# liznerski/eoe

Hardware: AMD Instinct MI355X
Metric: train images/sec, CLIP ViT-B/32 + HSC, 224x224 (higher is better)
Workload: dtype fp16; 1 GPU; CLIP ViT-B/32 (12 layers) + Linear(512,256) + HSC, full fine-tune, Adam lr 1e-4 wd 1e-3, 224x224, 128 normal + 128 OE images per GPU per step; global_batch=256, parallelism=dp1, launch=eager, weight-gradient launches on a side stream under the dgrad chain, arithmetic=16-bit MFMA operands, fp32 accumulate

## Files before the change

### eoe_amd/csrc/gemm.hip

```cpp
#include "gemm_common.h"
#include <stdlib.h>
#include <map>
#include <mutex>
#include <type_traits>

unsigned long long* g_stamp_buf = nullptr;
extern int g_tn_flags;
extern int g_vit_side_stream;
extern int g_attn_flags;
extern int g_tn256_launches;
extern int g_parity_flags;
int eoe_launch_nt256(const void* gemm_p, int dtype, int epi, int mi, hipStream_t s);
bool eoe_w8_applies(const void* gemm_p, int epi);
int eoe_launch_w8(const void* gemm_p, int dtype, int epi, hipStream_t s);
bool eoe_w8_streamk(const void* gemm_p);

namespace {
extern int g_nt_flags;


template <typename T, int EPI, int NI, int FLAGS, int GATHER = 0>
__global__ __launch_bounds__(512, 2) void gemm_nt_kernel(GemmP p) {
    extern __shared__ __attribute__((aligned(16))) char smem[];
    const int tid = threadIdx.x, lane = tid & 63, wave = tid >> 6;
// ... 660 lines not shown
        EOE_NT128_CASE(EOE_EPI_GELU_BWD)
        default: return eoe_set_error(EOE_ERR_ARG, "gemm_nt: unknown epilogue %d", epi);
    }
#undef EOE_NT128_CASE
    EOE_CHECK_LAUNCH("gemm_nt128");
    return finish_colsum(p, epi, MI, s);
}

template <typename T>
int launch_nt128w(const GemmP& p, int epi, hipStream_t s) {
    const int tiles = cdiv(p.M, 160) * cdiv(p.N, 256);
#define EOE_NT128W_CASE(E)                                                                  \
    case E:                                                                                 \
        { static bool once = (hipFuncSetAttribute((const void*)gemm_nt128w_kernel<T, E>, hipFuncAttributeMaxDynamicSharedMemorySize, SMEMW_BYTES), true); (void)once; } \
        hipLaunchKernelGGL((gemm_nt128w_kernel<T, E>), dim3(tiles), dim3(256), SMEMW_BYTES, s, p); \
        break;
    switch (epi) {
        EOE_NT128W_CASE(EOE_EPI_NONE)
        EOE_NT128W_CASE(EOE_EPI_GELU)
        EOE_NT128W_CASE(EOE_EPI_RESIDUAL)
        EOE_NT128W_CASE(EOE_EPI_GELU_BWD)
        default: return eoe_set_error(EOE_ERR_ARG, "gemm_nt: unknown epilogue %d", epi);
    }
#undef EOE_NT128W_CASE
    EOE_CHECK_LAUNCH("gemm_nt128w");
    return finish_colsum(p, epi, 5, s);
}

template <typename T>
int launch_nt128_auto(const GemmP& p, int epi, hipStream_t s) {
    const int slots = 2 * num_cus();
    const long t4 = (long)cdiv(p.M, 128) * cdiv(p.N, 128), t5 = (long)cdiv(p.M, 160) * cdiv(p.N, 128);
    const long c4 = (t4 + slots - 1) / slots * 128, c5 = (t5 + slots - 1) / slots * 160;
    const bool five = (g_nt_flags & 32) || (!(g_nt_flags & 16) && c5 <= c4);
    return five ? launch_nt128<T, 5>(p, epi, s) : launch_nt128<T, 4>(p, epi, s);
}

template <typename T>
__global__ __launch_bounds__(256) void nt_splitk_finish_kernel(const float* __restrict__ part, int S, int M, int N, float alpha,
                                                               const float* __restrict__ bias, const float* __restrict__ res, int ldres,
                                                               void* __restrict__ C, int ldc, int out_f32) {
    const int nq = N / 4;
    const int i = blockIdx.x * blockDim.x + threadIdx.x;
    if (i >= M * nq) return;
    const int m = i / nq, n = (i - m * nq) * 4;
    f32x4 v = *(const f32x4*)(part + (size_t)m * N + n);
    for (int s2 = 1; s2 < S; ++s2) v += *(const f32x4*)(part + ((size_t)s2 * M + m) * N + n);
    v *= alpha;
    if (bias) v += *(const f32x4*)(bias + n);
    if (res) v += *(const f32x4*)(res + (size_t)m * ldres + n);
    if (out_f32) *(f32x4*)((float*)C + (size_t)m * ldc + n) = v;
    else *(u32x2*)((T*)C + (size_t)m * ldc + n) = pack4<T>(v[0], v[1], v[2], v[3]);
}

template <typename T>
int launch_nt128_splitk(const GemmP& p, int epi, hipStream_t s) {
    const int nk = p.K / BK;
    if ((g_nt_flags & 8192) || !p.split_k || p.M > 1024 || nk < 24 || (epi != EOE_EPI_NONE && epi != EOE_EPI_RESIDUAL) || p.colsum || p.colsum_sq || p.accumulate ||
        (p.N & 15) || (p.ldc & 3) || (epi == EOE_EPI_RESIDUAL && (p.ldaux & 3)))
        return -1;
    int S = 8;
    while (S > 1 && (nk % S) != 0) S >>= 1;
    if (S < 2 || nk / S < 3) return -1;
    float* part = p.sk_part;
    if (!part || (size_t)S * p.M * p.N > (size_t)2 * num_cus() * 65536) return -1;
    GemmP q = p;
    q.C = part; q.ldc = p.N; q.out_f32 = 1; q.bias = nullptr; q.aux = nullptr; q.alpha = 1.0f;
    const int tiles = cdiv(p.M, 128) * cdiv(p.N, 128);
    { static bool once = (hipFuncSetAttribute((const void*)gemm_nt128_kernel<T, EOE_EPI_NONE, 4>, hipFuncAttributeMaxDynamicSharedMemorySize, smem128_bytes(4)), true); (void)once; }
    hipLaunchKernelGGL((gemm_nt128_kernel<T, EOE_EPI_NONE, 4>), dim3(tiles, S), dim3(256), smem128_bytes(4), s, q);
    EOE_CHECK_LAUNCH("gemm_nt128 (split k)");
    hipLaunchKernelGGL((nt_splitk_finish_kernel<T>), dim3(cdiv(p.M * (p.N / 4), 256)), dim3(256), 0, s, (const float*)part, S, p.M, p.N, p.alpha,
                       p.bias, epi == EOE_EPI_RESIDUAL ? (const float*)p.aux : nullptr, p.ldaux, p.C, p.ldc, p.out_f32);
    EOE_CHECK_LAUNCH("nt_splitk_finish");
    return 0;
}


int g_nt_flags = EOE_NT_DEFAULT_FLAGS;

template <typename T, int NI, int FLAGS>
int launch_nt_f(const GemmP& p, int epi, int grid, hipStream_t s) {
#define EOE_NT_CASE(E)                                                                      \
    case E:                                                                                 \
        { static bool once = (hipFuncSetAttribute((const void*)gemm_nt_kernel<T, E, NI, FLAGS>, hipFuncAttributeMaxDynamicSharedMemorySize, SMEM_BYTES), true); (void)once; } \
        hipLaunchKernelGGL((gemm_nt_kernel<T, E, NI, FLAGS>), dim3(grid), dim3(512), SMEM_BYTES, s, p); \
        break;
    switch (epi) {
        EOE_NT_CASE(EOE_EPI_NONE)
        EOE_NT_CASE(EOE_EPI_GELU)
        EOE_NT_CASE(EOE_EPI_RESIDUAL)
        EOE_NT_CASE(EOE_EPI_GELU_BWD)
        default: return eoe_set_error(EOE_ERR_ARG, "gemm_nt: unknown epilogue %d", epi);
    }
#undef EOE_NT_CASE
    EOE_CHECK_LAUNCH("gemm_nt");
    return finish_colsum(p, epi, 4, s);
}

template <typename T, int NI, int GATHER>
int launch_nt_conv(const GemmP& p, int grid, hipStream_t s) {
    static bool once = (hipFuncSetAttribute((const void*)gemm_nt_kernel<T, EOE_EPI_NONE, NI, EOE_NT_DEFAULT_FLAGS, GATHER>,
                                            hipFuncAttributeMaxDynamicSharedMemorySize, SMEM_BYTES), true);
    (void)once;
    hipLaunchKernelGGL((gemm_nt_kernel<T, EOE_EPI_NONE, NI, EOE_NT_DEFAULT_FLAGS, GATHER>), dim3(grid), dim3(512), SMEM_BYTES, s, p);
    EOE_CHECK_LAUNCH("gemm_nt");
    return finish_colsum(p, EOE_EPI_NONE, 4, s);
}

template <typename T, int NI>
int launch_nt_ni(const GemmP& p, int epi, int grid, hipStream_t s) {
#ifdef EOE_AB
    switch (g_nt_flags & 3) {
        case 0: return launch_nt_f<T, NI, 0>(p, epi, grid, s);
        case 1: return launch_nt_f<T, NI, 1>(p, epi, grid, s);
        case 2: return launch_nt_f<T, NI, 2>(p, epi, grid, s);
        default: return launch_nt_f<T, NI, 3>(p, epi, grid, s);
    }
#else
    return launch_nt_f<T, NI, EOE_NT_DEFAULT_FLAGS>(p, epi, grid, s);
#endif
}

template <typename T>
int launch_nt(const GemmP& p, int epi, int gather, hipStream_t s) {
    const int ncu = num_cus();
    if (epi == EOE_EPI_NONE && p.N <= 64 && (gather == 0 || gather == 1 || gather == 2) && !(g_nt_flags & 64)) {
        const int rc = gather == 2 ? launch_nt64<T, 2>(p, s) : (gather ? launch_nt64<T, 1>(p, s) : launch_nt64<T, 0>(p, s));
        return rc ? rc : finish_colsum(p, EOE_EPI_NONE, 4, s);
    }
    if (gather == 1 && epi == EOE_EPI_NONE && p.N >= 128 && !(g_nt_flags & 2048)) {
        const int slots = 2 * ncu;
        const long t4 = (long)cdiv(p.M, 128) * cdiv(p.N, 128), t5 = (long)cdiv(p.M, 160) * cdiv(p.N, 128);
        const long c4 = (t4 + slots - 1) / slots * 128, c5 = (t5 + slots - 1) / slots * 160;
        if (!p.colsum_sq && c5 < c4) return launch_nt128_gather<T, 5>(p, s);
        return launch_nt128_gather<T, 4>(p, s);
    }
    if (gather || (epi == EOE_EPI_NONE && p.N <= 64)) {
        const bool narrow = p.N <= 64;
        const int tiles = cdiv(p.M, BM) * cdiv(p.N, narrow ? 64 : 128);
        const int grid = tiles < ncu ? tiles : ncu;
        if (gather == 2) return narrow ? launch_nt_conv<T, 2, 2>(p, grid, s) : launch_nt_conv<T, 4, 2>(p, grid, s);
        if (gather == 3) return narrow ? launch_nt_conv<T, 2, 3>(p, grid, s) : launch_nt_conv<T, 4, 3>(p, grid, s);
        if (gather) return narrow ? launch_nt_conv<T, 2, 1>(p, grid, s) : launch_nt_conv<T, 4, 1>(p, grid, s);
        return launch_nt_conv<T, 2, 0>(p, grid, s);
    }
    if ((g_nt_flags & (128 | 256)) && epilogue_direct_ok(p, epi))
        return eoe_launch_nt256(&p, std::is_same<T, f16_t>::value ? EOE_F16 : EOE_BF16, epi, (g_nt_flags & 256) ? 8 : 5, s);
    const bool big = p.K >= 4096 && p.N >= 2048;
    if (gather == 0 && p.split_k) {
        const int rc = launch_nt128_splitk<T>(p, epi, s);
        if (rc >= 0) return rc;
    }
    if (!(g_nt_flags & (131072 | 4 | 8 | 512)) && gather == 0 && p.M >= 2048 && eoe_w8_applies(&p, epi)) {
        const long tiles = (long)cdiv(p.M, 256) * (p.N / 256);
        if ((g_nt_flags & 262144) || eoe_w8_streamk(&p) || tiles * 100 >= ((tiles + ncu - 1) / ncu) * ncu * 85) 
            return eoe_launch_w8(&p, std::is_same<T, f16_t>::value ? EOE_F16 : EOE_BF16, epi, s);
    }
    if (!(g_nt_flags & (4096 | 4 | 8 | 512)) && gather == 0 && !p.colsum_sq && (p.N % 256) == 0 && p.N >= 2048 && (p.K % 32) == 0 && p.M >= 2048) {
        const long tiles = (long)cdiv(p.M, 160) * (p.N / 256), slots = 2L * ncu;
        if (tiles * 10 >= ((tiles + slots - 1) / slots) * slots * 9) return launch_nt128w<T>(p, epi, s);
    }
    const bool gelu_wide = epi == EOE_EPI_GELU && p.N >= 2048 && p.K <= 1024 && !(g_nt_flags & 1024);
    if (((g_nt_flags & 512) || gelu_wide) && !(g_nt_flags & (4 | 8)) && epilogue_direct_ok(p, epi) && p.M >= 2048 && p.N >= 512) {
        const int nk = p.K / BK;
        long best = 0;
        int mi_best = 5;
        for (int mi : {5, 8}) {
            const long tiles = (long)cdiv(p.M, 32 * mi) * cdiv(p.N, 256);
            const long cost = ((tiles + ncu - 1) / ncu) * ((long)mi * (nk + 2) + 30);
            if (!best || cost < best) { best = cost; mi_best = mi; }
        }
        return eoe_launch_nt256(&p, std::is_same<T, f16_t>::value ? EOE_F16 : EOE_BF16, epi, mi_best, s);
    }
    if (big && !(g_nt_flags & (4 | 8)) && epilogue_direct_ok(p, epi) && p.M >= 2048)
        return eoe_launch_nt256(&p, std::is_same<T, f16_t>::value ? EOE_F16 : EOE_BF16, epi, 8, s);
    if (!p.colsum_sq && ((g_nt_flags & 8) || (!big && !(g_nt_flags & 4)))) return launch_nt128_auto<T>(p, epi, s);
    const int t4 = cdiv(p.M, BM) * cdiv(p.N, 128), t3 = cdiv(p.M, BM) * cdiv(p.N, 96);
    const int c4 = cdiv(t4, ncu) * 4, c3 = cdiv(t3, ncu) * 3;
    const int force = (g_nt_flags >> 4) & 7;
    const bool use3 = force ? (force == 3) : (c3 * 10 <= c4 * 9);
    const int tiles = use3 ? t3 : t4;
    const int grid = tiles < ncu ? tiles : ncu;
    return use3 ? launch_nt_ni<T, 3>(p, epi, grid, s) : launch_nt_ni<T, 4>(p, epi, grid, s);
}

int fill_params(const eoe_gemm_args* a, GemmP& p) {
    EOE_CHECK_ARG(a != nullptr, "gemm: null args");
    EOE_CHECK_ARG(a->A && a->B && a->C, "gemm: null operand");
    EOE_CHECK_ARG(a->M > 0 && a->N > 0 && a->K > 0, "gemm: bad shape %d %d %d", a->M, a->N, a->K);
    EOE_CHECK_ARG(a->dtype == EOE_F16 || a->dtype == EOE_BF16, "gemm: bad dtype %d", a->dtype);
    EOE_CHECK_ARG((a->lda % 8) == 0 && (a->ldb % 8) == 0, "gemm: lda/ldb must be multiples of 8 (16-B rows)");
    EOE_CHECK_ARG((((uintptr_t)a->A | (uintptr_t)a->B) & 15) == 0, "gemm: A/B must be 16-B aligned");
    EOE_CHECK_ARG(!a->accumulate || a->out_f32, "gemm: accumulate needs an fp32 C");
    p.A = a->A; p.B = a->B; p.C = a->C; p.bias = a->bias; p.aux = a->aux; p.aux_out = a->aux_out; p.colsum = a->colsum;
    p.colsum_part = nullptr; p.colsum_sq = 0; p.colsum_blocked = 0;
    p.M = a->M; p.N = a->N; p.K = a->K; p.lda = a->lda; p.ldb = a->ldb; p.ldc = a->ldc; p.ldaux = a->ldaux;
    p.out_f32 = a->out_f32; p.accumulate = a->accumulate; p.alpha = a->alpha; p.split_k = a->split_k;
    p.sk_part = nullptr; p.sk_sync = nullptr; p.sk_rounds = 0; p.sk_flags = 0;
    if (a->sk_workspace && a->sk_workspace_bytes >= (int64_t)EOE_NT_STREAMK_WORKSPACE_BYTES(num_cus()) && (((uintptr_t)a->sk_workspace) & 15) == 0) {
        p.sk_sync = (int*)a->sk_workspace;
        p.sk_part = (float*)((char*)a->sk_workspace + 8192);
    }
    EOE_CHECK_ARG((a->K % BK) == 0, "gemm_nt: K=%d must be a multiple of %d", a->K, BK);
    EOE_CHECK_ARG(a->ldb >= a->K, "gemm_nt: leading dims smaller than K");
    size_t ba = ((size_t)(a->M - 1) * a->lda + a->K) * 2;
    const size_t bb = ((size_t)(a->N - 1) * a->ldb + a->K) * 2;
    p.gH = p.gW = p.gC = p.gWo = p.gHoWo = p.gkw = p.gstride = p.gpad = p.gkstep = p.gkh = p.glog2c = 0;
    p.gmagic = 0;
    if (a->gather == 2) {
        const eoe_conv_geometry& g = a->geo;
        EOE_CHECK_ARG(a->epilogue == EOE_EPI_NONE, "gemm_nt: an implicit patch matrix supports the plain epilogue only");
        EOE_CHECK_ARG(g.n > 0 && g.C == 4 && g.kh > 0 && g.kw > 0 && g.kw <= 8 && g.stride > 0 && g.stride % 2 == 0 && g.pad == 0 && g.Ho > 0 &&
                      g.Wo > 0 && g.W % 2 == 0, "gemm_nt: bad packed first-layer geometry");
        EOE_CHECK_ARG((g.Ho - 1) * g.stride + g.kh <= g.H && (g.Wo - 1) * g.stride + 8 <= g.W && a->M == g.n * g.Ho * g.Wo &&
                      a->K == (g.kh + 1) / 2 * BK, "gemm_nt: packed geometry does not match M = %d, K = %d (image must be padded)", a->M, a->K);
        ba = (size_t)g.n * g.H * g.W * 4 * 2;
        p.gH = g.H; p.gW = g.W; p.gC = 4; p.gWo = g.Wo; p.gHoWo = g.Ho * g.Wo; p.gkw = g.kw; p.gstride = g.stride;
        p.gkstep = 2 * g.W * 8;
    } else if (a->gather) {
        const eoe_conv_geometry& g = a->geo;
        EOE_CHECK_ARG(a->epilogue == EOE_EPI_NONE, "gemm_nt: an implicit patch matrix supports the plain epilogue only");
        const bool narrowc = g.C == 8 || g.C == 16 || g.C == 32;
        EOE_CHECK_ARG(g.n > 0 && g.H > 0 && g.W > 0 && g.C > 0 && (g.C % BK == 0 || narrowc) && g.kh > 0 && g.kw > 0 && g.stride > 0 &&
                      g.pad >= 0 && g.Ho > 0 && g.Wo > 0, "gemm_nt: bad conv geometry (C = %d must be 8, 16, 32 or a multiple of %d)", g.C, BK);
        EOE_CHECK_ARG(a->M == g.n * g.Ho * g.Wo && (narrowc ? a->K >= g.kh * g.kw * g.C : a->K == g.kh * g.kw * g.C),
                      "gemm_nt: conv geometry does not match M = %d, K = %d", a->M, a->K);
        if (narrowc) {
            p.gkh = g.kh;
            p.glog2c = g.C == 8 ? 3 : (g.C == 16 ? 4 : 5);
            p.gmagic = (65536u + (unsigned)g.kw - 1) / (unsigned)g.kw;
            EOE_CHECK_ARG((a->K >> p.glog2c) < 4096, "gemm_nt: too many taps");
        }
        ba = (size_t)g.n * g.H * g.W * g.C * 2;
        p.gH = g.H; p.gW = g.W; p.gC = g.C; p.gWo = g.Wo; p.gHoWo = g.Ho * g.Wo; p.gkw = g.kw; p.gstride = g.stride; p.gpad = g.pad;
    } else {
        EOE_CHECK_ARG(a->lda >= a->K, "gemm_nt: leading dims smaller than K");
    }
    EOE_CHECK_ARG(ba < 0x7fffffffull && bb < 0x7fffffffull, "gemm: operand larger than 2 GiB");
    p.bytesA = (unsigned)ba; p.bytesB = (unsigned)bb;
    static const int dbg = getenv("EOE_GEMM_DEBUG") ? atoi(getenv("EOE_GEMM_DEBUG")) : 0;
    if (dbg & 1) { p.bytesA = 0; p.bytesB = 0; }
    p.dbg = dbg | ((g_nt_flags & 524288) ? 32 : 0) | ((g_nt_flags & 8388608) ? 64 : 0);
    p.stamp = nullptr;
    static const int stampon = getenv("EOE_GEMM_STAMP") ? atoi(getenv("EOE_GEMM_STAMP")) : 0;
    if (stampon) {
        static unsigned long long* buf = [] { void* b = nullptr; (void)hipMalloc(&b, 4096 * 16 * 8); return (unsigned long long*)b; }();
        (void)hipMemsetAsync(buf, 0, 4096 * 16 * 8, 0);
        p.stamp = buf;
        g_stamp_buf = buf;
    }
    if (a->epilogue == EOE_EPI_GELU) EOE_CHECK_ARG(!a->out_f32, "gemm: the GELU epilogue needs a 16-bit C");
    if (a->epilogue == EOE_EPI_RESIDUAL) EOE_CHECK_ARG(a->aux && a->out_f32, "gemm: RESIDUAL epilogue needs aux, fp32 C");
    if (a->epilogue == EOE_EPI_GELU_BWD) EOE_CHECK_ARG(a->aux, "gemm: GELU_BWD epilogue needs aux");
    return 0;
}

}

int eoe_nt_flags() { return g_nt_flags; }

extern "C" int eoe_gemm_nt(const eoe_gemm_args* a, void* stream) {
    GemmP p;
    EOE_TRY(fill_params(a, p));
    const int osz = a->out_f32 ? 4 : 2;
    static const bool by_shape = getenv("EOE_PROF_SHAPES") != nullptr;
    char pname[32] = "gemm_nt";
    if (by_shape) snprintf(pname, sizeof(pname), "nt_%dx%dx%d_e%d%s", a->M, a->N, a->K, a->epilogue, a->colsum ? "c" : "");
    ProfScope ps(pname, 2.0 * a->M * a->N * a->K,
                 2.0 * ((a->gather ? (double)a->geo.n * a->geo.H * a->geo.W * a->geo.C : (double)a->M * a->K) + (double)a->N * a->K) +
                     (double)osz * a->M * a->N *
                     (a->epilogue == EOE_EPI_GELU ? 2 : 1) + (a->epilogue == EOE_EPI_RESIDUAL ? 4.0 * a->M * a->N : 0.0) +
                     (a->epilogue == EOE_EPI_GELU_BWD ? 2.0 * a->M * a->N : 0.0), stream);
    const int mode = (a->gather == 1 && p.gkh) ? 3 : a->gather;
    if (a->colsum && a->workspace && a->workspace_bytes >= (int64_t)EOE_NT_COLSUM_WORKSPACE_BYTES(a->M, a->N))
        p.colsum_part = (float*)a->workspace, p.colsum_blocked = ((a->N & 63) == 0 && (a->N & 3) == 0) ? 1 : 0;
    if (a->colstats) {
        EOE_CHECK_ARG(a->epilogue != EOE_EPI_GELU && !a->colsum, "gemm_nt: colstats goes with neither the GELU epilogue nor colsum");
        EOE_CHECK_ARG(a->workspace && a->workspace_bytes >= 2 * (int64_t)EOE_NT_COLSUM_WORKSPACE_BYTES(a->M, a->N),
                      "gemm_nt: colstats needs a workspace of 2 * EOE_NT_COLSUM_WORKSPACE_BYTES(M, N)");
        EOE_CHECK_ARG((a->N & 15) == 0 && (a->ldc & 7) == 0 && (a->ldaux & 7) == 0 && (((uintptr_t)a->C) & 15) == 0,
                      "gemm_nt: colstats needs N %% 16 == 0 and 16-byte aligned rows of C");
        p.colsum_part = (float*)a->workspace;
        p.colsum_sq = 1;
        p.colsum_blocked = 0;
    }
    return a->dtype == EOE_F16 ? launch_nt<f16_t>(p, a->epilogue, mode, (hipStream_t)stream)
                               : launch_nt<bf16_t>(p, a->epilogue, mode, (hipStream_t)stream);
}


extern "C" int eoe_debug_gemm_stamps(unsigned long long* out, int n_words) {
    if (!g_stamp_buf || !out) return eoe_set_error(EOE_ERR_ARG, "gemm stamps are not enabled (EOE_GEMM_STAMP=1)");
    if (hipDeviceSynchronize() != hipSuccess) return eoe_set_error(EOE_ERR_LAUNCH, "sync failed");
    if (hipMemcpy(out, g_stamp_buf, (size_t)n_words * 8, hipMemcpyDeviceToHost) != hipSuccess)
        return eoe_set_error(EOE_ERR_LAUNCH, "copy failed");
    return 0;
}

extern "C" int eoe_set_option(const char* name, int value) {
    if (name && !strcmp(name, "nt_flags")) { g_nt_flags = value; return 0; }
    if (name && !strcmp(name, "tn_flags")) { g_tn_flags = value; return 0; }
    if (name && !strcmp(name, "vit_side_stream")) { g_vit_side_stream = value; return 0; }
    if (name && !strcmp(name, "attn_flags")) { g_attn_flags = value; return 0; }
    if (name && !strcmp(name, "parity_flags")) { g_parity_flags = value; return 0; }
    return eoe_set_error(EOE_ERR_ARG, "unknown option");
}

extern "C" int eoe_get_option(const char* name, int* value) {
// ... 10 lines not shown
```

### eoe_amd/csrc/gemm_w8.hip

```cpp
#include "gemm_common.h"
#include <type_traits>

int eoe_nt_flags();

namespace {

constexpr int W8_A_BYTES = 256 * BK * 2;
constexpr int W8_STAGE_BYTES = 2 * W8_A_BYTES;
constexpr int W8_NST = 2;
constexpr int W8_BIAS_OFF = W8_NST * W8_STAGE_BYTES;
constexpr int W8_SYNC_OFF = W8_BIAS_OFF + 2 * 1024;
constexpr int W8_SMEM_BYTES = W8_SYNC_OFF + 64;
static_assert(W8_SMEM_BYTES <= 160 * 1024, "LDS");

#define W8_A10(n) "a" #n "0", "a" #n "1", "a" #n "2", "a" #n "3", "a" #n "4", "a" #n "5", "a" #n "6", "a" #n "7", "a" #n "8", "a" #n "9"
#define W8_AGPRS "a0", "a1", "a2", "a3", "a4", "a5", "a6", "a7", "a8", "a9", W8_A10(1), W8_A10(2), W8_A10(3), W8_A10(4), W8_A10(5), W8_A10(6), \
    W8_A10(7), W8_A10(8), W8_A10(9), W8_A10(10), W8_A10(11), "a120", "a121", "a122", "a123", "a124", "a125", "a126", "a127"
#define W8_MFMA_INPLACE(MNEM, E, A, B) asm volatile(MNEM " a[%c0:%c1], %2, %3, a[%c0:%c1]" :: "i"(4 * (E)), "i"(4 * (E) + 3), "v"(A), "v"(B) : W8_AGPRS)
#define W8_MFMA_FIRST(MNEM, E, A, B) asm volatile(MNEM " a[%c0:%c1], %2, %3, 0" :: "i"(4 * (E)), "i"(4 * (E) + 3), "v"(A), "v"(B) : W8_AGPRS)

#ifndef W8_ST_AUX
#define W8_ST_AUX 0
#endif
template <int N> __device__ __forceinline__ void w8_wait_vm() {
    static_assert(N >= 0 && N <= 63, "vmcnt");
    asm volatile("s_waitcnt vmcnt(%0)" :: "n"(N) : "memory");
}

template <typename T, int EPI, bool SK>
__global__ __launch_bounds__(512, 2) void gemm_w8_kernel(GemmP p) {
    static_assert(EPI == EOE_EPI_NONE || EPI == EOE_EPI_GELU, "epilogues with a second input are not built yet");
    constexpr int A_B = W8_A_BYTES, STAGE = W8_STAGE_BYTES, NST = W8_NST;
    constexpr int PER = 8;
    constexpr int NMF = 32;
    constexpr int NB = 8;
    constexpr int ES = (EPI == EOE_EPI_GELU) ? 2 : 1;
    constexpr int L = (EPI == EOE_EPI_GELU) ? 66 : 13;
    extern __shared__ __attribute__((aligned(16))) char smem[];
    asm volatile("" ::: W8_AGPRS);
    const int tid = threadIdx.x, lane = tid & 63;
    const unsigned wave_u = (unsigned)__builtin_amdgcn_readfirstlane(tid >> 6);
    const int tiles_n = p.N >> 8;
    const int total_tiles = tiles_n * ((p.M + 255) >> 8);
    const int G = gridDim.x;
    const int nk = p.K / BK;
    const int xcd = (int)blockIdx.x & 7, wq = (int)blockIdx.x >> 3, Wn = G >> 3;
    const int sk_R = SK ? p.sk_rounds : 0;
    const int sk_Ix = SK ? ((total_tiles - sk_R * G - xcd + 7) >> 3) * nk : 0;
    auto sk_bound = [&](int i) -> int {
        int v = (int)(((long long)i * sk_Ix) / Wn);
        const int m = v % nk;
        if (m == 1) v -= 1;
        else if (m == nk - 1) v += 1;
        return v;
    };
    auto sk_wg_of = [&](int v) -> int {
        int g = (int)(((long long)v * Wn) / (sk_Ix > 0 ? sk_Ix : 1));
        if (g > Wn - 1) g = Wn - 1;
        while (g + 1 < Wn && sk_bound(g + 1) <= v) ++g;
        while (g > 0 && sk_bound(g) > v) --g;
        return g;
    };
    const int sk_lo = SK ? sk_bound(wq) : 0, sk_hi = SK ? sk_bound(wq + 1) : 0;
    const int sk_t0 = sk_lo / nk;
    const int n_sk = sk_hi > sk_lo ? (sk_hi - 1) / nk - sk_t0 + 1 : 0;
    const int my_tiles = SK ? sk_R + n_sk : (total_tiles - (int)blockIdx.x + G - 1) / G;
    const int iters = SK ? sk_R * nk + (sk_hi - sk_lo) : my_tiles * nk;
    if (iters <= 0) return;
    const bool sk_first = SK && (p.sk_flags & 1);
    const unsigned lds0 = (unsigned)(uintptr_t)((lds_void_t*)smem);
    auto seg_get = [&](int j, int& vb, int& kb, int& ke, int& js) {
        js = -1;
        if (SK) {
            const bool is_sk = sk_first ? (j < n_sk) : (j >= sk_R);
            if (is_sk) {
                js = sk_first ? j : j - sk_R;
                const int t = sk_t0 + js;
                kb = js == 0 ? sk_lo - sk_t0 * nk : 0;
                ke = sk_hi - t * nk < nk ? sk_hi - t * nk : nk;
                vb = sk_R * G + t * 8 + xcd;
                return;
            }
            if (sk_first) j -= n_sk;
        }
        vb = (int)blockIdx.x + j * G;
        kb = 0;
        ke = nk;
    };
    auto tile_of = [&](int vb, int& m0, int& n0) {
        const int r = xcd_remap(vb, total_tiles);
        m0 = (r / tiles_n) * 256;
        n0 = (r % tiles_n) * 256;
    };

    __amdgpu_buffer_rsrc_t ra = make_rsrc(p.A, p.bytesA);
    __amdgpu_buffer_rsrc_t rb = make_rsrc(p.B, p.bytesB);
    __amdgpu_buffer_rsrc_t rbias = make_rsrc(p.bias ? (const void*)p.bias : p.C, p.bias ? (unsigned)p.N * 4u : 0u);
    const int l8 = lane >> 3;
    unsigned voffA[2], voffB[2];
#pragma unroll
    for (int par = 0; par < 2; ++par) {
        const int c = (lane & 7) ^ ((par * 4 + (lane >> 4)) & 7);
        voffA[par] = (unsigned)((l8 * p.lda + c * 8) * 2);
        voffB[par] = (unsigned)((((lane >> 5) * 8 + (l8 & 3)) * p.ldb + c * 8) * 2);
    }
    int st_tile = 0, st_kt = 0, st_kb = 0, st_kend = nk, st_slot = 0;
    unsigned sA_base = 0, sB_base = 0, bias_vo = EOE_OOB;
    int rows_left = 0;
    auto set_offsets = [&](int t) {
        int m0, n0, vb, js;
        seg_get(t, vb, st_kb, st_kend, js);
        st_kt = st_kb;
        tile_of(vb, m0, n0);
        if (p.dbg & 4) m0 = 0;
        if (p.dbg & 8) n0 = 0;
        const int ra0 = m0 + (int)wave_u * 32;
        sA_base = (unsigned)ra0 * (unsigned)p.lda * 2u;
        rows_left = p.M - ra0;
        sB_base = (unsigned)(n0 + (int)wave_u * 32) * (unsigned)p.ldb * 2u;
        bias_vo = (unsigned)((n0 + lane * 4) * 4);
    };
#define W8_DMA16(rsrc, lds_addr, voff, soff)                                                                          \
    asm volatile("s_mov_b32 m0, %0\n\ts_nop 0\n\tbuffer_load_dwordx4 %1, %2, %3 offen lds"                           \
                 :: "s"(lds_addr), "v"(voff), "s"(rsrc), "s"(soff) : "memory")
    auto stage_piece = [&](int j, bool live) {
        const unsigned sa = lds0 + (unsigned)st_slot * STAGE;
        const unsigned k0 = (unsigned)st_kt * (BK * 2u);
        if (j < 4) {
            const unsigned la = sa + (wave_u * 4 + j) * 1024u;
            const unsigned vo = (live && l8 + j * 8 < rows_left) ? voffA[j & 1] : EOE_OOB;
            const unsigned so = sA_base + (unsigned)(j * 8) * (unsigned)p.lda * 2u + k0;
            W8_DMA16(ra, la, vo, so);
        } else {
            const int jb = j - 4;
            const unsigned lb = sa + A_B + (wave_u * 4 + jb) * 1024u;
            const unsigned so = sB_base + (unsigned)((jb & 1) * 16 + ((jb >> 1) & 1) * 4) * (unsigned)p.ldb * 2u + k0;
            const unsigned vo = live ? voffB[jb & 1] : EOE_OOB;
            W8_DMA16(rb, lb, vo, so);
        }
    };
    auto stage_bias = [&](bool live) {
        if (live && wave_u == 0 && st_kt == st_kb) {
            const unsigned la = lds0 + (unsigned)W8_BIAS_OFF + (unsigned)(st_tile & 1) * 1024u;
            W8_DMA16(rbias, la, bias_vo, 0);
        }
    };
    auto stage_advance = [&]() {
        st_slot ^= 1;
        if (++st_kt == st_kend) {
            st_tile += 1;
            if (st_tile < my_tiles) set_offsets(st_tile);
        }
    };

    const int wm0 = (int)(wave_u >> 2) * 128, wn0 = (int)(wave_u & 3) * 64;
    const int lr = lane & 15, lg = lane >> 4;
    const int sw = (lr >> 1) & 7;
    const int fragA = (wm0 + lr) * 128, fragB = A_B + (wn0 + lr) * 128;
    const int ch0 = ((0 + lg) ^ sw) * 16, ch1 = ((4 + lg) ^ sw) * 16;
    typedef typename T16<T>::v8 V8;
    const unsigned c_bytes = (unsigned)((((size_t)p.M - 1) * p.ldc + p.N) * 2);
    __amdgpu_buffer_rsrc_t rc = make_rsrc(p.C, c_bytes);
    __amdgpu_buffer_rsrc_t rpre = make_rsrc(p.aux_out ? p.aux_out : p.C, p.aux_out ? c_bytes : 0u);
    const float alpha = p.alpha;
    const int ldc2 = p.ldc * 2;
    const unsigned lane_off = (unsigned)(lr * ldc2 + lg * 16);
#define W8_CLUSTER(FIRST, STAGEP, LIVE, READS, WBC, WBN, rbase, rks)                                                          \
    do {                                                                                                         \
        const unsigned ra_ = (unsigned)(size_t)((rbase) - smem) + fragA + ((rks) ? ch1 : ch0);                   \
        const unsigned rb_ = (unsigned)(size_t)((rbase) - smem) + fragB + ((rks) ? ch1 : ch0);                   \
        _Pragma("unroll") for (int mi = 0; mi < 8; ++mi) {                                                       \
            if (mi == 0) asm volatile("s_waitcnt lgkmcnt(7)" : "+v"(xa[0]), "+v"(WBC[0]), "+v"(WBC[1]), "+v"(WBC[2]), "+v"(WBC[3]) :: "memory"); \
            else asm volatile("s_waitcnt lgkmcnt(11)" : "+v"(xa[mi]) :: "memory");                              \
            __builtin_amdgcn_sched_barrier(0);                                                                   \
            _Pragma("unroll") for (int ni = 0; ni < 4; ++ni) {                                                   \
                const int e_ = mi * 4 + ni;                                                                      \
                if (std::is_same<T, f16_t>::value) {                                                             \
                    if (FIRST) W8_MFMA_FIRST("v_mfma_f32_16x16x32_f16", e_, WBC[ni], xa[mi]);                    \
                    else W8_MFMA_INPLACE("v_mfma_f32_16x16x32_f16", e_, WBC[ni], xa[mi]);                        \
                } else {                                                                                         \
                    if (FIRST) W8_MFMA_FIRST("v_mfma_f32_16x16x32_bf16", e_, WBC[ni], xa[mi]);                   \
                    else W8_MFMA_INPLACE("v_mfma_f32_16x16x32_bf16", e_, WBC[ni], xa[mi]);                       \
                }                                                                                                \
                if ((READS) && mi == 0) asm volatile("ds_read_b128 %0, %1 offset:%2" : "=v"(WBN[ni]) : "v"(rb_), "i"(ni * 2048)); \
            }                                                                                                    \
            if (READS) asm volatile("ds_read_b128 %0, %1 offset:%2" : "=v"(xa[mi]) : "v"(ra_), "i"(mi * 2048)); \
            if (STAGEP) stage_piece(mi, LIVE);                                                                     \
        }                                                                                                        \
    } while (0)
#define W8_ITER(FIRST, LASTK)                                                                                    \
    do {                                                                                                         \
        const char* sc = smem + cur * STAGE;                                                                     \
        const char* sn = smem + (cur ^ 1) * STAGE;                                                               \
        W8_CLUSTER(FIRST, false, false, true, wb0, wb1, sc, 1);                                                  \
        if ((FIRST) && c_tile > 0) w8_wait_vm<NB * 2 * ES>(); else w8_wait_vm<0>();                              \
        asm volatile("s_waitcnt lgkmcnt(0)" : "+v"(xa[0]), "+v"(xa[1]), "+v"(xa[2]), "+v"(xa[3]), "+v"(xa[4]), "+v"(xa[5]), "+v"(xa[6]), \
                     "+v"(xa[7]), "+v"(wb1[0]), "+v"(wb1[1]), "+v"(wb1[2]), "+v"(wb1[3]) :: "memory");           \
        __builtin_amdgcn_sched_barrier(0);                                                                       \
        __builtin_amdgcn_s_barrier();                                                                            \
        const bool live_ = it + 2 < iters;                                                                       \
        stage_bias(live_);                                                                                       \
        W8_CLUSTER(false, true, live_, !(LASTK), wb1, wb0, sn, 0);                                               \
        if (live_) stage_advance();                                                                              \
        cur ^= 1;                                                                                                \
        ++it;                                                                                                    \
    } while (0)

    V8 xa[8], wb0[4], wb1[4];
    int cur = 0, it = 0;
    set_offsets(0);
#pragma unroll 1
    for (int i = 0; i < 2; ++i) {
        stage_bias(true);
#pragma unroll
        for (int j = 0; j < PER; ++j) stage_piece(j, true);
        stage_advance();
    }
    w8_wait_vm<PER>();
    __builtin_amdgcn_s_barrier();
#define W8_FIRST_FRAGS()                                                                                         \
    do {                                                                                                         \
        const unsigned a_ = (unsigned)(cur * STAGE) + fragA + ch0, b_ = (unsigned)(cur * STAGE) + fragB + ch0;   \
        _Pragma("unroll") for (int i = 0; i < 4; ++i) asm volatile("ds_read_b128 %0, %1 offset:%2" : "=v"(wb0[i]) : "v"(b_), "i"(i * 2048)); \
        _Pragma("unroll") for (int i = 0; i < 8; ++i) asm volatile("ds_read_b128 %0, %1 offset:%2" : "=v"(xa[i]) : "v"(a_), "i"(i * 2048)); \
    } while (0)
    __amdgpu_buffer_rsrc_t rpart = make_rsrc(SK ? (const void*)p.sk_part : p.C, SK ? (unsigned)(2 * G) * 262144u : 0u);
    const unsigned part_voff = (unsigned)lane * 16u;
    auto part_store = [&](int slot) {
        const int so = slot * 262144 + (int)wave_u * 32768;
#pragma unroll
        for (int e = 0; e < 32; ++e)
            asm volatile("buffer_store_dwordx4 a[%c0:%c1], %2, %3, %4 offen sc1" :: "i"(4 * e), "i"(4 * e + 3), "v"(part_voff), "s"(rpart), "s"(so + e * 1024) : "memory");
    };
    auto part_load = [&](int slot) {
        const int so = slot * 262144 + (int)wave_u * 32768;
#pragma unroll
        for (int e = 0; e < 32; ++e)
            asm volatile("buffer_load_dwordx4 a[%c0:%c1], %2, %3, %4 offen sc1" :: "i"(4 * e), "i"(4 * e + 3), "v"(part_voff), "s"(rpart), "s"(so + e * 1024) : "memory", W8_AGPRS);
        asm volatile("s_waitcnt vmcnt(0)" ::: "memory", W8_AGPRS);
    };
    auto part_add = [&](int slot) {
        const int so = slot * 262144 + (int)wave_u * 32768;
        constexpr int DEPTH = 8;
        f32x4 ld[DEPTH];
#pragma unroll
        for (int e = 0; e < DEPTH; ++e) ld[e] = __builtin_bit_cast(f32x4, __builtin_amdgcn_raw_buffer_load_b128(rpart, (int)part_voff, so + e * 1024, 16));
#pragma unroll
        for (int e = 0; e < 32; ++e) {
            const f32x4 v = ld[e % DEPTH];
#pragma unroll
            for (int r = 0; r < 4; ++r) {
                float a;
                asm volatile("v_accvgpr_read_b32 %0, a[%c1]" : "=v"(a) : "i"(4 * e + r));
                a += v[r];
                asm volatile("v_accvgpr_write_b32 a[%c0], %1" :: "i"(4 * e + r), "v"(a) : W8_AGPRS);
            }
            if (e + DEPTH < 32) ld[e % DEPTH] = __builtin_bit_cast(f32x4, __builtin_amdgcn_raw_buffer_load_b128(rpart, (int)part_voff, so + (e + DEPTH) * 1024, 16));
        }
    };
    for (int c_tile = 0; c_tile < my_tiles; ++c_tile) {
        int c_vb, c_kb, c_ke, c_js;
        seg_get(c_tile, c_vb, c_kb, c_ke, c_js);
        W8_FIRST_FRAGS();
        W8_ITER(true, false);
        _Pragma("unroll 1") for (int kt = c_kb + 1; kt < c_ke - 1; ++kt) W8_ITER(false, false);
        W8_ITER(false, true);
        int m0, n0;
        tile_of(c_vb, m0, n0);
        asm volatile("s_nop 15\n\ts_nop 15" ::: "memory");
        __builtin_amdgcn_sched_barrier(0);
        if (SK && c_ke - c_kb < nk) {
            const int t = sk_t0 + c_js;
            const int w_first = sk_wg_of(t * nk), w_last = sk_wg_of(t * nk + nk - 1);
            const int S = w_last - w_first + 1, me = wq - w_first;
            int* arrive = p.sk_sync + (t * 8 + xcd);
            int* flags = p.sk_sync + 1024;
            const int my_slot = (int)blockIdx.x * 2 + (c_js == 0 ? 0 : 1);
            auto slot_of = [&](int sgm) -> int {
                const int wc = w_first + sgm;
                return (wc * 8 + xcd) * 2 + ((sgm > 0 || sk_bound(wc) >= t * nk) ? 0 : 1);
            };
            volatile int* sw = (volatile int*)(smem + W8_SYNC_OFF);
            if (tid == 0) sw[0] = __hip_atomic_fetch_add(arrive, 1, __ATOMIC_RELAXED, __HIP_MEMORY_SCOPE_AGENT);
            __syncthreads();
            const bool owner = __builtin_amdgcn_readfirstlane(sw[0]) == S - 1;
            if (!owner) {
                part_store(my_slot);
                asm volatile("s_waitcnt vmcnt(0)" ::: "memory");
                __syncthreads();
                if (tid == 0) __hip_atomic_store(flags + my_slot, 1, __ATOMIC_RELAXED, __HIP_MEMORY_SCOPE_AGENT);
                continue;
            }
            if (me >= 2) {
                part_store(my_slot);
                asm volatile("s_waitcnt vmcnt(0)" ::: "memory");
            }
            if (tid == 0) {
                __hip_atomic_store(arrive, 0, __ATOMIC_RELAXED, __HIP_MEMORY_SCOPE_AGENT);
                int bad = 0;
                for (int sgm = 0; sgm < S; ++sgm) {
                    if (sgm == me) continue;
                    int* f = flags + slot_of(sgm);
                    int spins = 0;
                    while (__hip_atomic_load(f, __ATOMIC_RELAXED, __HIP_MEMORY_SCOPE_AGENT) != 1 && ++spins < (1 << 22)) __builtin_amdgcn_s_sleep(4);
                    if (spins >= (1 << 22)) bad = 1;
                    __hip_atomic_store(f, 0, __ATOMIC_RELAXED, __HIP_MEMORY_SCOPE_AGENT);
                }
                sw[1] = bad;
            }
            __syncthreads();
            const bool poisoned = __builtin_amdgcn_readfirstlane(sw[1]) != 0;
            if (me >= 2) part_load(slot_of(0));
            for (int sgm = me >= 2 ? 1 : 0; sgm < S; ++sgm) {
                if (me < 2 && sgm == me) continue;
                part_add(sgm == me ? my_slot : slot_of(sgm));
            }
            if (poisoned) {
                const float qnan = __builtin_nanf("");
#pragma unroll
                for (int e = 0; e < 128; ++e) asm volatile("v_accvgpr_write_b32 a[%c0], %1" :: "i"(e), "v"(qnan) : W8_AGPRS);
            }
            asm volatile("s_nop 7" ::: "memory");
        }
        float bias16[16];
        float cv[8], xv[8], wv[8];
        V8 hv = {}, av = {};
#pragma unroll
        for (int c = 0; c < 8; ++c) cv[c] = 0.f;
        auto load_cv = [&](const int band, const int q) {
#pragma unroll
            for (int b = 0; b < NB; ++b) {
                if (band == b) {
#pragma unroll
                    for (int e = 0; e < 2; ++e)
#pragma unroll
                        for (int r = 0; r < 4; ++r)
                            asm volatile("v_accvgpr_read_b32 %0, a[%c1]" : "=v"(cv[4 * e + r]) : "i"(4 * (b * 4 + 2 * q + e) + r));
                }
            }
        };
        auto load_bias16 = [&](unsigned slot) {
#pragma unroll
            for (int qq = 0; qq < 2; ++qq)
#pragma unroll
                for (int e = 0; e < 2; ++e) {
                    const f32x4 bv = *(const f32x4*)(smem + slot + (unsigned)((wn0 + qq * 32 + lg * 8 + e * 4) * 4));
#pragma unroll
                    for (int r = 0; r < 4; ++r) bias16[qq * 8 + e * 4 + r] = bv[r];
                }
        };
        unsigned e_voff = EOE_OOB;
        int e_soff = 0;
        constexpr float C1702 = -1.702f * 1.4426950408889634f;
        auto epi_op = [&](const int q, const int k) {
            if (k < 8) {
                xv[k] = cv[k] * alpha + bias16[8 * q + k];
                asm volatile("" : "+v"(xv[k]));
                return;
            }
            if (k < 12) { const int j = k - 8; hv[2 * j] = (T)xv[2 * j]; hv[2 * j + 1] = (T)xv[2 * j + 1]; return; }
            if (k == 12) {
                if (EPI == EOE_EPI_GELU) __builtin_amdgcn_raw_buffer_store_b128(__builtin_bit_cast(u32x4, hv), rpre, (int)e_voff, e_soff + q * 64, W8_ST_AUX);
                else __builtin_amdgcn_raw_buffer_store_b128(__builtin_bit_cast(u32x4, hv), rc, (int)e_voff, e_soff + q * 64, W8_ST_AUX);
                return;
            }
            if (EPI != EOE_EPI_GELU) return;
            if (k < 21) { const int j = k - 13; xv[j] = (float)hv[j]; return; }
            if (k < 29) { const int j = k - 21; wv[j] = C1702 * xv[j]; return; }
            if (k < 37) { const int j = k - 29; wv[j] = __builtin_amdgcn_exp2f(wv[j]); return; }
            if (k < 45) { const int j = k - 37; wv[j] = 1.0f + wv[j]; return; }
            if (k < 53) { const int j = k - 45; wv[j] = __builtin_amdgcn_rcpf(wv[j]); return; }
            if (k < 61) { const int j = k - 53; wv[j] = xv[j] * wv[j]; return; }
            if (k < 65) { const int j = k - 61; av[2 * j] = (T)wv[2 * j]; av[2 * j + 1] = (T)wv[2 * j + 1]; return; }
            if (k == 65) __builtin_amdgcn_raw_buffer_store_b128(__builtin_bit_cast(u32x4, av), rc, (int)e_voff, e_soff + q * 64, W8_ST_AUX);
        };

        load_bias16((unsigned)W8_BIAS_OFF + (unsigned)(c_tile & 1) * 1024u);
        _Pragma("unroll 1") for (int band = 0; band < NB; ++band) {
            const int mrow = m0 + wm0 + band * 16;
            e_voff = (mrow + lr < p.M) ? lane_off : EOE_OOB;
            e_soff = mrow * ldc2 + (n0 + wn0) * 2;
            load_cv(band, 0);
#pragma unroll
            for (int k = 0; k < L; ++k) epi_op(0, k);
            load_cv(band, 1);
#pragma unroll
            for (int k = 0; k < L; ++k) epi_op(1, k);
        }
    }
#undef W8_ITER
#undef W8_FIRST_FRAGS
#undef W8_CLUSTER
#undef W8_DMA16
}

int w8_sk_rounds(const GemmP& p, int tiles, int ncu) {
    const int g_nt_flags = eoe_nt_flags();
    if (!(g_nt_flags & 1048576) || !p.sk_part || !p.sk_sync || (ncu & 7) || ncu > 256 || tiles <= 0) return -1;
    const int nk = p.K / BK;
    if (nk < 4 || tiles % ncu == 0) return -1;
    int R = tiles / ncu;
    if ((g_nt_flags & 2097152) && R >= 1) R -= 1;
    const int tsk = tiles - R * ncu;
    if (tsk < 8 || (long)(tsk / 8) * nk < 4L * (ncu / 8)) return -1;
    return R;
}

template <typename T>
int launch_w8(const GemmP& p0, int epi, hipStream_t s) {
    GemmP p = p0;
    const int tiles = cdiv(p.M, 256) * (p.N / 256);
    const int ncu = num_cus();
    const int R = w8_sk_rounds(p, tiles, ncu);
    const bool sk = R >= 0;
    const int grid = sk ? ncu : (tiles < ncu ? tiles : ncu);
    p.sk_rounds = sk ? R : 0;
    p.sk_flags = (eoe_nt_flags() & 4194304) ? 1 : 0;
#define EOE_W8_LAUNCH(E, SK_)                                                               \
    do {                                                                                    \
        static bool once = (hipFuncSetAttribute((const void*)gemm_w8_kernel<T, E, SK_>, hipFuncAttributeMaxDynamicSharedMemorySize, W8_SMEM_BYTES), true); (void)once; \
        hipLaunchKernelGGL((gemm_w8_kernel<T, E, SK_>), dim3(grid), dim3(512), W8_SMEM_BYTES, s, p); \
    } while (0)
#define EOE_W8_CASE(E)                                                                      \
    case E:                                                                                 \
        if (sk) EOE_W8_LAUNCH(E, true); else EOE_W8_LAUNCH(E, false);                       \
        break;
    switch (epi) {
        EOE_W8_CASE(EOE_EPI_NONE)
        EOE_W8_CASE(EOE_EPI_GELU)
        default: return eoe_set_error(EOE_ERR_ARG, "gemm_w8: epilogue %d is not built", epi);
    }
#undef EOE_W8_CASE
#undef EOE_W8_LAUNCH
    EOE_CHECK_LAUNCH("gemm_w8");
    return 0;
}

}

bool eoe_w8_applies(const void* gemm_p, int epi) {
    const GemmP& p = *(const GemmP*)gemm_p;
    if (epi != EOE_EPI_NONE && epi != EOE_EPI_GELU) return false;
    if (p.out_f32 || p.accumulate || p.colsum || p.colsum_part || p.colsum_sq || p.split_k) return false;
    if ((p.N & 255) || (p.K % BK) || p.K / BK < 2 || p.M < 256) return false;
    if (!epilogue_fast_ok(p)) return false;
    const size_t c_bytes = (((size_t)p.M - 1) * p.ldc + p.N) * 2 + (size_t)256 * p.ldc * 2;
    const size_t a_reach = ((size_t)p.M + 256) * p.lda * 2 + (size_t)p.K * 2;
    return c_bytes < 0x7fffffffull && a_reach < 0x7fffffffull;
}

bool eoe_w8_streamk(const void* gemm_p) {
    const GemmP& p = *(const GemmP*)gemm_p;
    return w8_sk_rounds(p, cdiv(p.M, 256) * (p.N / 256), num_cus()) >= 0;
}

int eoe_launch_w8(const void* gemm_p, int dtype, int epi, hipStream_t s) {
    const GemmP& p = *(const GemmP*)gemm_p;
#ifdef EOE_W8_DEV
    return launch_w8<f16_t>(p, epi, s);
#else
    return dtype == EOE_F16 ? launch_w8<f16_t>(p, epi, s) : launch_w8<bf16_t>(p, epi, s);
#endif
}
```

Measured before the change: 25760 images/sec.

## Split tail-round tiles into half-height tiles in w8 GEMM

Adds a tail variant of the 256x256 w8 GEMM kernel. When the last wave of tiles fills at most half the CUs, each leftover tile is split into two 128-row halves that run on separate workgroups, so the final partial round finishes sooner. This needs half-height staging offsets, a 4-fragment MFMA cluster path and a half-band epilogue. The dispatch heuristic gains an optional flag that counts half rounds, and the minimum M in the applicability check is relaxed. The cost is more code paths, extra per-tile branching, and lower MFMA efficiency on the half tiles.

```diff
diff --git a/eoe_amd/csrc/gemm.hip b/eoe_amd/csrc/gemm.hip
--- a/eoe_amd/csrc/gemm.hip
+++ b/eoe_amd/csrc/gemm.hip
@@ -836,9 +836,12 @@
         const int rc = launch_nt128_splitk<T>(p, epi, s);
         if (rc >= 0) return rc;
     }
-    if (!(g_nt_flags & (131072 | 4 | 8 | 512)) && gather == 0 && p.M >= 2048 && eoe_w8_applies(&p, epi)) {
+    if (!(g_nt_flags & (131072 | 4 | 8 | 512)) && gather == 0 && (p.M >= 2048 || (g_nt_flags & 262144)) && eoe_w8_applies(&p, epi)) {
         const long tiles = (long)cdiv(p.M, 256) * (p.N / 256);
-        if ((g_nt_flags & 262144) || eoe_w8_streamk(&p) || tiles * 100 >= ((tiles + ncu - 1) / ncu) * ncu * 85) 
+        const long tail = tiles % ncu;
+        const bool cut = (g_nt_flags & 33554432) && !(g_nt_flags & 16777216) && tail > 0 && 2 * tail <= ncu;
+        const long half_rounds = 2 * (tiles / ncu) + (tail == 0 ? 0 : cut ? 1 : 2);
+        if ((g_nt_flags & 262144) || eoe_w8_streamk(&p) || 2 * tiles * 100 >= half_rounds * ncu * 85)
             return eoe_launch_w8(&p, std::is_same<T, f16_t>::value ? EOE_F16 : EOE_BF16, epi, s);
     }
     if (!(g_nt_flags & (4096 | 4 | 8 | 512)) && gather == 0 && !p.colsum_sq && (p.N % 256) == 0 && p.N >= 2048 && (p.K % 32) == 0 && p.M >= 2048) {
diff --git a/eoe_amd/csrc/gemm_w8.hip b/eoe_amd/csrc/gemm_w8.hip
--- a/eoe_amd/csrc/gemm_w8.hip
+++ b/eoe_amd/csrc/gemm_w8.hip
@@ -27,8 +27,8 @@
     asm volatile("s_waitcnt vmcnt(%0)" :: "n"(N) : "memory");
 }
 
-template <typename T, int EPI, bool SK>
-__global__ __launch_bounds__(512, 2) void gemm_w8_kernel(GemmP p) {
+template <typename T, int EPI, bool SK, bool TAIL>
+__device__ __forceinline__ void w8_body(const GemmP& p) {
     static_assert(EPI == EOE_EPI_NONE || EPI == EOE_EPI_GELU, "epilogues with a second input are not built yet");
     constexpr int A_B = W8_A_BYTES, STAGE = W8_STAGE_BYTES, NST = W8_NST;
     constexpr int PER = 8;
@@ -64,7 +64,14 @@
     const int sk_lo = SK ? sk_bound(wq) : 0, sk_hi = SK ? sk_bound(wq + 1) : 0;
     const int sk_t0 = sk_lo / nk;
     const int n_sk = sk_hi > sk_lo ? (sk_hi - 1) / nk - sk_t0 + 1 : 0;
-    const int my_tiles = SK ? sk_R + n_sk : (total_tiles - (int)blockIdx.x + G - 1) / G;
+    const int full_r = total_tiles / G, tail = total_tiles - full_r * G;
+    const bool split = TAIL && !SK && !(p.sk_flags & 2) && tail > 0 && 2 * tail <= G;
+    const int half_t = (G & 15) ? (int)blockIdx.x >> 1 : ((wq >> 1) << 3) + xcd;
+    const int half_h = (G & 15) ? (int)blockIdx.x & 1 : wq & 1;
+    const int half_vb = full_r * G + half_t;
+    const bool has_half = split && half_t < tail && (xcd_remap(half_vb, total_tiles) / tiles_n) * 256 + half_h * 128 < p.M;
+    const int my_tiles = SK ? sk_R + n_sk : split ? full_r + (has_half ? 1 : 0) : (total_tiles - (int)blockIdx.x + G - 1) / G;
+    auto seg_half = [&](int j) -> bool { return TAIL && !SK && has_half && j == full_r; };
     const int iters = SK ? sk_R * nk + (sk_hi - sk_lo) : my_tiles * nk;
     if (iters <= 0) return;
     const bool sk_first = SK && (p.sk_flags & 1);
@@ -83,7 +90,7 @@
             }
             if (sk_first) j -= n_sk;
         }
-        vb = (int)blockIdx.x + j * G;
+        vb = seg_half(j) ? half_vb : (int)blockIdx.x + j * G;
         kb = 0;
         ke = nk;
     };
@@ -107,6 +114,8 @@
     int st_tile = 0, st_kt = 0, st_kb = 0, st_kend = nk, st_slot = 0;
     unsigned sA_base = 0, sB_base = 0, bias_vo = EOE_OOB;
     int rows_left = 0;
+    bool st_half = false;
+    unsigned st_a_lds = wave_u * 4096u, st_a_skip = 0;
     auto set_offsets = [&](int t) {
         int m0, n0, vb, js;
         seg_get(t, vb, st_kb, st_kend, js);
@@ -114,9 +123,13 @@
         tile_of(vb, m0, n0);
         if (p.dbg & 4) m0 = 0;
         if (p.dbg & 8) n0 = 0;
-        const int ra0 = m0 + (int)wave_u * 32;
+        st_half = seg_half(t);
+        const int ra0 = st_half ? m0 + half_h * 128 + (int)wave_u * 16 : m0 + (int)wave_u * 32;
         sA_base = (unsigned)ra0 * (unsigned)p.lda * 2u;
         rows_left = p.M - ra0;
+        if (st_half && rows_left > 16) rows_left = 16;
+        st_a_lds = st_half ? wave_u * 2048u : wave_u * 4096u;
+        st_a_skip = st_half ? 16384u - 2048u : 0u;
         sB_base = (unsigned)(n0 + (int)wave_u * 32) * (unsigned)p.ldb * 2u;
         bias_vo = (unsigned)((n0 + lane * 4) * 4);
     };
@@ -127,7 +140,7 @@
         const unsigned sa = lds0 + (unsigned)st_slot * STAGE;
         const unsigned k0 = (unsigned)st_kt * (BK * 2u);
         if (j < 4) {
-            const unsigned la = sa + (wave_u * 4 + j) * 1024u;
+            const unsigned la = sa + st_a_lds + (unsigned)j * 1024u + (j >= 2 ? st_a_skip : 0u);
             const unsigned vo = (live && l8 + j * 8 < rows_left) ? voffA[j & 1] : EOE_OOB;
             const unsigned so = sA_base + (unsigned)(j * 8) * (unsigned)p.lda * 2u + k0;
             W8_DMA16(ra, la, vo, so);
@@ -157,6 +170,7 @@
     const int lr = lane & 15, lg = lane >> 4;
     const int sw = (lr >> 1) & 7;
     const int fragA = (wm0 + lr) * 128, fragB = A_B + (wn0 + lr) * 128;
+    const int wm0h = (int)(wave_u >> 2) * 64;
     const int ch0 = ((0 + lg) ^ sw) * 16, ch1 = ((4 + lg) ^ sw) * 16;
     typedef typename T16<T>::v8 V8;
     const unsigned c_bytes = (unsigned)((((size_t)p.M - 1) * p.ldc + p.N) * 2);
@@ -165,13 +179,15 @@
     const float alpha = p.alpha;
     const int ldc2 = p.ldc * 2;
     const unsigned lane_off = (unsigned)(lr * ldc2 + lg * 16);
-#define W8_CLUSTER(FIRST, STAGEP, LIVE, READS, WBC, WBN, rbase, rks)                                                          \
+#define W8_CLUSTER(MR, FA, FIRST, STAGEP, LIVE, READS, WBC, WBN, rbase, rks)                                     \
     do {                                                                                                         \
-        const unsigned ra_ = (unsigned)(size_t)((rbase) - smem) + fragA + ((rks) ? ch1 : ch0);                   \
+        const unsigned ra_ = (unsigned)(size_t)((rbase) - smem) + (FA) + ((rks) ? ch1 : ch0);                    \
         const unsigned rb_ = (unsigned)(size_t)((rbase) - smem) + fragB + ((rks) ? ch1 : ch0);                   \
-        _Pragma("unroll") for (int mi = 0; mi < 8; ++mi) {                                                       \
-            if (mi == 0) asm volatile("s_waitcnt lgkmcnt(7)" : "+v"(xa[0]), "+v"(WBC[0]), "+v"(WBC[1]), "+v"(WBC[2]), "+v"(WBC[3]) :: "memory"); \
-            else asm volatile("s_waitcnt lgkmcnt(11)" : "+v"(xa[mi]) :: "memory");                              \
+        _Pragma("unroll") for (int mi = 0; mi < (MR); ++mi) {                                                    \
+            if (mi == 0 && (MR) == 8) asm volatile("s_waitcnt lgkmcnt(7)" : "+v"(xa[0]), "+v"(WBC[0]), "+v"(WBC[1]), "+v"(WBC[2]), "+v"(WBC[3]) :: "memory"); \
+            else if (mi == 0) asm volatile("s_waitcnt lgkmcnt(3)" : "+v"(xa[0]), "+v"(WBC[0]), "+v"(WBC[1]), "+v"(WBC[2]), "+v"(WBC[3]) :: "memory"); \
+            else if ((MR) == 8) asm volatile("s_waitcnt lgkmcnt(11)" : "+v"(xa[mi]) :: "memory");               \
+            else asm volatile("s_waitcnt lgkmcnt(7)" : "+v"(xa[mi]) :: "memory");                               \
             __builtin_amdgcn_sched_barrier(0);                                                                   \
             _Pragma("unroll") for (int ni = 0; ni < 4; ++ni) {                                                   \
                 const int e_ = mi * 4 + ni;                                                                      \
@@ -185,22 +201,28 @@
                 if ((READS) && mi == 0) asm volatile("ds_read_b128 %0, %1 offset:%2" : "=v"(WBN[ni]) : "v"(rb_), "i"(ni * 2048)); \
             }                                                                                                    \
             if (READS) asm volatile("ds_read_b128 %0, %1 offset:%2" : "=v"(xa[mi]) : "v"(ra_), "i"(mi * 2048)); \
-            if (STAGEP) stage_piece(mi, LIVE);                                                                     \
+            if ((STAGEP) && (MR) == 8) stage_piece(mi, LIVE);                                                    \
+            if ((STAGEP) && (MR) == 4 && mi < 2) stage_piece(mi, LIVE);                                          \
+            if ((STAGEP) && (MR) == 4) stage_piece(mi + 4, LIVE);                                                \
         }                                                                                                        \
     } while (0)
-#define W8_ITER(FIRST, LASTK)                                                                                    \
+#define W8_ITER(MR, FA, FIRST, LASTK)                                                                            \
     do {                                                                                                         \
         const char* sc = smem + cur * STAGE;                                                                     \
         const char* sn = smem + (cur ^ 1) * STAGE;                                                               \
-        W8_CLUSTER(FIRST, false, false, true, wb0, wb1, sc, 1);                                                  \
+        W8_CLUSTER(MR, FA, FIRST, false, false, true, wb0, wb1, sc, 1);                                          \
         if ((FIRST) && c_tile > 0) w8_wait_vm<NB * 2 * ES>(); else w8_wait_vm<0>();                              \
-        asm volatile("s_waitcnt lgkmcnt(0)" : "+v"(xa[0]), "+v"(xa[1]), "+v"(xa[2]), "+v"(xa[3]), "+v"(xa[4]), "+v"(xa[5]), "+v"(xa[6]), \
-                     "+v"(xa[7]), "+v"(wb1[0]), "+v"(wb1[1]), "+v"(wb1[2]), "+v"(wb1[3]) :: "memory");           \
+        if ((MR) == 8)                                                                                           \
+            asm volatile("s_waitcnt lgkmcnt(0)" : "+v"(xa[0]), "+v"(xa[1]), "+v"(xa[2]), "+v"(xa[3]), "+v"(xa[4]), "+v"(xa[5]), "+v"(xa[6]), \
+                         "+v"(xa[7]), "+v"(wb1[0]), "+v"(wb1[1]), "+v"(wb1[2]), "+v"(wb1[3]) :: "memory");       \
+        else                                                                                                     \
+            asm volatile("s_waitcnt lgkmcnt(0)" : "+v"(xa[0]), "+v"(xa[1]), "+v"(xa[2]), "+v"(xa[3]), "+v"(wb1[0]), "+v"(wb1[1]), "+v"(wb1[2]), \
+                         "+v"(wb1[3]) :: "memory");                                                              \
         __builtin_amdgcn_sched_barrier(0);                                                                       \
         __builtin_amdgcn_s_barrier();                                                                            \
         const bool live_ = it + 2 < iters;                                                                       \
         stage_bias(live_);                                                                                       \
-        W8_CLUSTER(false, true, live_, !(LASTK), wb1, wb0, sn, 0);                                               \
+        W8_CLUSTER(MR, FA, false, true, live_, !(LASTK), wb1, wb0, sn, 0);                                       \
         if (live_) stage_advance();                                                                              \
         cur ^= 1;                                                                                                \
         ++it;                                                                                                    \
@@ -218,11 +240,11 @@
     }
     w8_wait_vm<PER>();
     __builtin_amdgcn_s_barrier();
-#define W8_FIRST_FRAGS()                                                                                         \
+#define W8_FIRST_FRAGS(MR, FA)                                                                                   \
     do {                                                                                                         \
-        const unsigned a_ = (unsigned)(cur * STAGE) + fragA + ch0, b_ = (unsigned)(cur * STAGE) + fragB + ch0;   \
+        const unsigned a_ = (unsigned)(cur * STAGE) + (FA) + ch0, b_ = (unsigned)(cur * STAGE) + fragB + ch0;    \
         _Pragma("unroll") for (int i = 0; i < 4; ++i) asm volatile("ds_read_b128 %0, %1 offset:%2" : "=v"(wb0[i]) : "v"(b_), "i"(i * 2048)); \
-        _Pragma("unroll") for (int i = 0; i < 8; ++i) asm volatile("ds_read_b128 %0, %1 offset:%2" : "=v"(xa[i]) : "v"(a_), "i"(i * 2048)); \
+        _Pragma("unroll") for (int i = 0; i < (MR); ++i) asm volatile("ds_read_b128 %0, %1 offset:%2" : "=v"(xa[i]) : "v"(a_), "i"(i * 2048)); \
     } while (0)
     __amdgpu_buffer_rsrc_t rpart = make_rsrc(SK ? (const void*)p.sk_part : p.C, SK ? (unsigned)(2 * G) * 262144u : 0u);
     const unsigned part_voff = (unsigned)lane * 16u;
@@ -261,10 +283,19 @@
     for (int c_tile = 0; c_tile < my_tiles; ++c_tile) {
         int c_vb, c_kb, c_ke, c_js;
         seg_get(c_tile, c_vb, c_kb, c_ke, c_js);
-        W8_FIRST_FRAGS();
-        W8_ITER(true, false);
-        _Pragma("unroll 1") for (int kt = c_kb + 1; kt < c_ke - 1; ++kt) W8_ITER(false, false);
-        W8_ITER(false, true);
+        const bool c_half = seg_half(c_tile);
+        if (!c_half) {
+            W8_FIRST_FRAGS(8, fragA);
+            W8_ITER(8, fragA, true, false);
+            _Pragma("unroll 1") for (int kt = c_kb + 1; kt < c_ke - 1; ++kt) W8_ITER(8, fragA, false, false);
+            W8_ITER(8, fragA, false, true);
+        } else {
+            const int fragAh = (wm0h + lr) * 128;
+            W8_FIRST_FRAGS(4, fragAh);
+            W8_ITER(4, fragAh, true, false);
+            _Pragma("unroll 1") for (int kt = c_kb + 1; kt < c_ke - 1; ++kt) W8_ITER(4, fragAh, false, false);
+            W8_ITER(4, fragAh, false, true);
+        }
         int m0, n0;
         tile_of(c_vb, m0, n0);
         asm volatile("s_nop 15\n\ts_nop 15" ::: "memory");
@@ -376,8 +407,10 @@
         };
 
         load_bias16((unsigned)W8_BIAS_OFF + (unsigned)(c_tile & 1) * 1024u);
-        _Pragma("unroll 1") for (int band = 0; band < NB; ++band) {
-            const int mrow = m0 + wm0 + band * 16;
+        const int e_nb = c_half ? NB / 2 : NB;
+        const int e_m0 = m0 + (c_half ? half_h * 128 + wm0h : wm0);
+        _Pragma("unroll 1") for (int band = 0; band < e_nb; ++band) {
+            const int mrow = e_m0 + band * 16;
             e_voff = (mrow + lr < p.M) ? lane_off : EOE_OOB;
             e_soff = mrow * ldc2 + (n0 + wn0) * 2;
             load_cv(band, 0);
@@ -393,6 +426,11 @@
 #undef W8_CLUSTER
 #undef W8_DMA16
 }
+
+template <typename T, int EPI, bool SK>
+__global__ __launch_bounds__(512, 2) void gemm_w8_kernel(GemmP p) { w8_body<T, EPI, SK, false>(p); }
+template <typename T, int EPI>
+__global__ __launch_bounds__(512, 2) void gemm_w8_tail_kernel(GemmP p) { w8_body<T, EPI, false, true>(p); }
 
 int w8_sk_rounds(const GemmP& p, int tiles, int ncu) {
     const int g_nt_flags = eoe_nt_flags();
@@ -413,9 +451,12 @@
     const int ncu = num_cus();
     const int R = w8_sk_rounds(p, tiles, ncu);
     const bool sk = R >= 0;
-    const int grid = sk ? ncu : (tiles < ncu ? tiles : ncu);
+    const bool no_split = sk || (eoe_nt_flags() & 16777216);
+    const int grid = sk ? ncu : (tiles < ncu ? (!no_split && 2 * tiles <= ncu ? ncu : tiles) : ncu);
     p.sk_rounds = sk ? R : 0;
-    p.sk_flags = (eoe_nt_flags() & 4194304) ? 1 : 0;
+    p.sk_flags = ((eoe_nt_flags() & 4194304) ? 1 : 0) | (no_split ? 2 : 0);
+    const int tail = tiles % grid;
+    const bool cut = !no_split && tail > 0 && 2 * tail <= grid;
 #define EOE_W8_LAUNCH(E, SK_)                                                               \
     do {                                                                                    \
         static bool once = (hipFuncSetAttribute((const void*)gemm_w8_kernel<T, E, SK_>, hipFuncAttributeMaxDynamicSharedMemorySize, W8_SMEM_BYTES), true); (void)once; \
@@ -423,7 +464,11 @@
     } while (0)
 #define EOE_W8_CASE(E)                                                                      \
     case E:                                                                                 \
-        if (sk) EOE_W8_LAUNCH(E, true); else EOE_W8_LAUNCH(E, false);                       \
+        if (sk) EOE_W8_LAUNCH(E, true);                                                     \
+        else if (cut) {                                                                     \
+            static bool once = (hipFuncSetAttribute((const void*)gemm_w8_tail_kernel<T, E>, hipFuncAttributeMaxDynamicSharedMemorySize, W8_SMEM_BYTES), true); (void)once; \
+            hipLaunchKernelGGL((gemm_w8_tail_kernel<T, E>), dim3(grid), dim3(512), W8_SMEM_BYTES, s, p); \
+        } else EOE_W8_LAUNCH(E, false);                                                     \
         break;
     switch (epi) {
         EOE_W8_CASE(EOE_EPI_NONE)
@@ -442,7 +487,7 @@
     const GemmP& p = *(const GemmP*)gemm_p;
     if (epi != EOE_EPI_NONE && epi != EOE_EPI_GELU) return false;
     if (p.out_f32 || p.accumulate || p.colsum || p.colsum_part || p.colsum_sq || p.split_k) return false;
-    if ((p.N & 255) || (p.K % BK) || p.K / BK < 2 || p.M < 256) return false;
+    if ((p.N & 255) || (p.K % BK) || p.K / BK < 2 || p.M < 1) return false;
     if (!epilogue_fast_ok(p)) return false;
     const size_t c_bytes = (((size_t)p.M - 1) * p.ldc + p.N) * 2 + (size_t)256 * p.ldc * 2;
     const size_t a_reach = ((size_t)p.M + 256) * p.lda * 2 + (size_t)p.K * 2;
```

Result: no change. 25680 images/sec (-0.3%).
